# tbrown122387/ssme

Measured on AMD Instinct MI355X. Metric: particle-steps/sec (NxT) univ-SVOL bootstrap filter; log-lik delta vs CPU ref, higher is better.
Workload: dtype f64

## Files before the change

ssme_amd/csrc/pf_api.hip:

```cpp
#include "../../include/ssme_pf.h"
#include "pf_kernels.h"
#include "lw_kernels.h"
#include "pf_small.h"
#include "lw_small.h"
#include "user_expect.h"
#include "forecast.h"
#include "smooth.h"
#include "series_history.h"
#include "handle_core.h"
#include "shard_driver.h"

#include <cmath>
#include <cstdio>
#include <cstdlib>
#include <chrono>
#include <cstring>
#include <new>
#include <string>
#include <vector>

using namespace ssme;

struct StepKernels { const void* fn[2][2][3]; const void* wide[2]; int nt; };

struct ssme_pf_s : HandleCore {
    ssme_pf_config cfg;
    StepKernels kern;
    bool params_set;
    int debug_anc, keep_logw;
    int graph_mode;
    double *l2_T, *l2_R;
    double* l2_work;
    int32_t *l2_lo, *l2_hi;
    int32_t* l2_ticket;
    int l2_tables;
    double* small_ms;
    double* yz_step;
    int32_t* ticket;
    int num_cus;
    int small_series;
    double y_step_v[3];
    double z_step_v[3];
    int dx, dy;
    int kcov, kz;
    int nt;
    double *sh_x[2], *sh_c[2], *sh_loc, *sh_tsum, *sh_tmax, *sh_winx, *sh_winc;
    int sh_path;
    double* x[2];
    double* cdf[2];
    double* tsum[2];
    double* tmax[2];
    double *logw, *scratchR;
    double *exp_part, *exp_out;
    double* wscratch;
    double *uexp_part, *uexp_out;
    double last_z;
    double last_zv[kMaxCov];
    double* fc_zfut;
    size_t fc_zfut_cap;
    double *gam, *pgam, *gtot;
    uint32_t* anc;
    FilterScalars* scal;
    ModelConst* mc;
    int cur;
    hipGraphExec_t gexec;
    int g_T, g_has_z, g_debug, g_logw, g_nt;
    FunctionalIds g_rec_fs;
    int g_rec_user;
    FunctionalIds rec_fs;
    int rec_user;
    double *traj, *utraj;
    int traj_cap, traj_n;
    int rec_T, rec_n, rec_nh;
    SeriesHistoryState hist;
    double* hist_x;
    uint32_t* hist_anc;
// ... 162 lines not shown
                hipMemcpy(hs.data(), g_stamps, hs.size() * 8, hipMemcpyDeviceToHost);
                FILE* f = fopen(getenv("SSME_STAMPS_DUMP"), "w");
                for (size_t i = 0; i < hs.size(); i += 16) { for (int k = 0; k < 16; ++k) fprintf(f, "%llu ", hs[i + k]); fprintf(f, "\n"); }
                fclose(f);
            }
        }
    }
#endif
    return a;
}

static int default_tile(int n_particles, int n_filters) {
    if (n_particles <= kTile) return kTile;
    const long R = n_filters;
    if (R * ((n_particles + kTileSmall - 1) / kTileSmall) <= 256) return kTileSmall;
    if (R * ((n_particles + kTileMid - 1) / kTileMid) <= 512) return kTileMid;
    return kTile;
}

template <class F>
static void with_model(int model, F&& f) {
    switch (model) {
        case SSME_MODEL_SVOL: f(std::integral_constant<int, MODEL_SVOL>{}); break;
        case SSME_MODEL_SVOL_LEVERAGE: f(std::integral_constant<int, MODEL_SVOL_LEVERAGE>{}); break;
#if SSME_HAS_USER_MODEL
        case SSME_MODEL_USER0: f(std::integral_constant<int, MODEL_USER0>{}); break;
#endif
        default: f(std::integral_constant<int, MODEL_LIN_GAUSS>{}); break;
    }
}

template <int MODEL, int NT, int TILE, bool BIG, bool WL2>
static void fill_rs(const void* (&fn)[3]) {
    fn[0] = reinterpret_cast<const void*>(&k_filter_step<MODEL, NT, BIG, TILE, -1, WL2>);
    fn[1] = reinterpret_cast<const void*>(&k_filter_step<MODEL, NT, BIG, TILE, 0, WL2>);
    fn[2] = reinterpret_cast<const void*>(&k_filter_step<MODEL, NT, BIG, TILE, 1, WL2>);
}
template <int MODEL, int NT, int TILE>
static void fill_step_kernels(StepKernels& k) {
    k.nt = NT;
    fill_rs<MODEL, NT, TILE, false, false>(k.fn[0][0]);
    fill_rs<MODEL, NT, TILE, false, true>(k.fn[0][1]);
    fill_rs<MODEL, NT, TILE, true, false>(k.fn[1][0]);
}
template <int MODEL>
static StepKernels step_kernels(int tile) {
    StepKernels k{};
    if (tile == kTileSmall) fill_step_kernels<MODEL, 256, kTileSmall>(k);
    else if (tile == kTileMid) fill_step_kernels<MODEL, 512, kTileMid>(k);
    else {
        fill_step_kernels<MODEL, 512, kTile>(k);
        k.wide[0] = reinterpret_cast<const void*>(&k_filter_step<MODEL, 256, false, kTile, -1>);
        k.wide[1] = reinterpret_cast<const void*>(&k_filter_step<MODEL, 1024, false, kTile, -1>);
    }
    return k;
}
static hipError_t grant_step_lds(const ssme_pf_s* h) {
    hipError_t e = hipSuccess;
    for (int big = 0; big < 2; ++big)
        for (int wl2 = 0; wl2 < 2; ++wl2)
            for (const void* fn : h->kern.fn[big][wl2])
                if (fn && e == hipSuccess) e = grant_lds(fn, big ? h->lds_bytes_big : h->lds_bytes, h->cfg.device);
    for (const void* fn : h->kern.wide)
        if (fn && e == hipSuccess) e = grant_lds(fn, h->lds_bytes, h->cfg.device);
    return e;
}

struct StepLaunch { const void* fn; int nt; size_t lds; };
static StepLaunch select_step_kernel(const ssme_pf_s* h, const StepArgs& a) {
    int rs = -1;
    if (h->cfg.resamp_sched == 1 && a.t > 0 && !a.anc && !a.logw && !a.ticket)
        rs = h->cfg.resampler == SSME_RESAMP_MULTINOMIAL ? 0 : (h->cfg.resampler == SSME_RESAMP_SYSTEMATIC ? 1 : -1);
    if (h->split_l2) return {h->kern.fn[1][0][rs + 1], h->kern.nt, h->lds_bytes_big};
    if (h->tile == kTile && h->nt != 512) return {h->kern.wide[h->nt == 1024], h->nt, h->lds_bytes};
    return {h->kern.fn[0][a.B <= 128 ? 1 : 0][rs + 1], h->kern.nt, h->lds_bytes};
}
static void launch_step_on(ssme_pf_handle h, const StepArgs& a, dim3 grid) {
    const StepLaunch k = select_step_kernel(h, a);
    void* args[] = {const_cast<StepArgs*>(&a)};
    hipLaunchKernel(k.fn, grid, dim3(k.nt), args, k.lds, h->stream);
}
static void launch_step(ssme_pf_handle h, const StepArgs& a) { launch_step_on(h, a, dim3(h->B, h->R)); }
static void launch_gamma(ssme_pf_handle h, int t0, int nT) {
    if (h->cfg.resampler != SSME_RESAMP_MULTINOMIAL) return;
    launch_gamma_tables(h, h->gam, h->pgam, h->gtot, STREAM_GAMMA, STREAM_RESAMP_EXTRA, h->tile, h->cfg.first_filter_id, t0, nT);
}
static void launch_level2(hipStream_t st, const StepArgs& a, int n_filters, size_t lds, int ranges) {
    if (a.l2_inkernel) {
        hipLaunchKernelGGL(k_l2_scan_blocks, dim3((a.B + 1023) / 1024, n_filters), dim3(1024), 0, st, a);
    } else if (a.l2_work && a.B > 1024) {
        const dim3 grid((a.B + 1023) / 1024, n_filters);
        hipLaunchKernelGGL(k_l2_scan_blocks, grid, dim3(1024), 0, st, a);
        hipLaunchKernelGGL(k_l2_ranges, grid, dim3(1024), lds, st, a, ranges);
    } else
        hipLaunchKernelGGL(k_level2_plan, dim3(n_filters), dim3(1024), lds, st, a, ranges);
}
static void launch_plan(ssme_pf_handle h, int t, int gi, bool plan_ranges, bool finalize_prev, bool record_per_step,
                        double* ll_host = nullptr) {
    StepArgs a = step_args(h);
    a.t = t; a.gi = gi; a.finalize_prev = finalize_prev ? 1 : 0;
    a.ll_host = ll_host;
    a.per_step = record_per_step ? h->per_step : nullptr;
    launch_level2(h->stream, a, h->R, h->lds_bytes_plan, plan_ranges ? 1 : 0);
}
static void launch_kf(ssme_pf_handle h, int t, bool record_per_step, double* ll_host = nullptr) {
    if (h->split_l2) { launch_plan(h, t + 1, 0, false, true, record_per_step, ll_host); return; }
    StepArgs a = step_args(h);
    a.ll_host = ll_host;
    a.t = t;
    a.per_step = record_per_step ? h->per_step : nullptr;
    hipLaunchKernelGGL(kf_finalize, dim3(h->R), dim3(kThreads), 0, h->stream, a);
}

static double* hist_row(const ssme_pf_s* h, int t) { return h->hist_x + (size_t)t * h->dx * h->R * h->Npad; }

static void enqueue_step(ssme_pf_handle h, int t, int yi, int gi, bool has_z, bool finalize_prev, bool record_per_step,
                         bool from_step_staging = false, bool results_to_host = true) {
    StepArgs a = step_args(h);
    a.z = has_z ? h->zbuf : nullptr;
    if (from_step_staging) {
        a.by_value = 1; a.y_now = h->pin[PinLayout::yz]; a.z_now = has_z ? h->pin[PinLayout::yz + 1] : 0.0;
        for (int d = 1; d < h->dy; ++d) a.y_now_v[d - 1] = h->y_step_v[d - 1];
        for (int j = 1; j < h->kcov; ++j) a.z_now_v[j - 1] = has_z ? h->z_step_v[j - 1] : 0.0;
        if (!h->split_l2) { a.ticket = h->ticket; a.ll_host = results_to_host ? h->pin_dev + PinLayout::results : nullptr; }
    }
    a.per_step = record_per_step ? h->per_step : nullptr;
    a.t = t; a.yi = yi; a.gi = gi; a.finalize_prev = finalize_prev ? 1 : 0;
// ... 2265 lines not shown
```

ssme_amd/csrc/pf_kernels.h:

```cpp
#pragma once
#include "ssme_math.h"
#include "model_api.h"

namespace ssme {

typedef unsigned long long u64;

constexpr int kThreads = 256;
constexpr int kWave = 64;
constexpr int kRow = 512;
constexpr int kTile = 2048;
constexpr int kTileSmall = 512;
constexpr int kTileMid = 1024;
constexpr int kMaxTilesPerFilter = 2048;
constexpr int kSplitLevel2Above = 1024;
constexpr int kL2Scratch = 64;
constexpr int kL2Offsets = 32;
constexpr int kMaxTilesSplit = 16384;
#ifndef SSME_SEARCH_WINDOW
#define SSME_SEARCH_WINDOW 16
#endif
constexpr int kStageTiles = 3;
constexpr int kEShift = 35;
constexpr int kTileShift = 41;
// ... 60 lines not shown
    int32_t* l2_lo;
    int32_t* l2_hi;
    double* l2_work;
    int32_t l2_inkernel;
    int32_t* l2_ticket;
    const double* l2_tsrc;
    const double* l2_offs;
    int32_t l2_offs_stride;
    int32_t prio_mode;
    int32_t stream_stores;
    const uint32_t* keyp;
    uint32_t first_filter;
    double logN;
    int32_t ablate;
    unsigned long long* stamps;
};

template <int CTRL, int ROWMASK>
__device__ __forceinline__ double dpp_f64_neginf(double v) {
    const u64 b = d2bits(v);
    const int lo = __builtin_amdgcn_update_dpp(0, (int)(uint32_t)b, CTRL, ROWMASK, 0xF, false);
    const int hi = __builtin_amdgcn_update_dpp((int)0xfff00000, (int)(uint32_t)(b >> 32), CTRL, ROWMASK, 0xF, false);
    return bits2d(((u64)(uint32_t)hi << 32) | (u64)(uint32_t)lo);
}
template <int CTRL, int ROWMASK>
__device__ __forceinline__ double dpp_f64_zero(double v) {
    const u64 b = d2bits(v);
    int lo, hi;
    if (ROWMASK == 0xF) {
        lo = __builtin_amdgcn_mov_dpp((int)(uint32_t)b, CTRL, 0xF, 0xF, true);
        hi = __builtin_amdgcn_mov_dpp((int)(uint32_t)(b >> 32), CTRL, 0xF, 0xF, true);
    } else {
        lo = __builtin_amdgcn_update_dpp(0, (int)(uint32_t)b, CTRL, ROWMASK, 0xF, false);
        hi = __builtin_amdgcn_update_dpp(0, (int)(uint32_t)(b >> 32), CTRL, ROWMASK, 0xF, false);
    }
    return bits2d(((u64)(uint32_t)hi << 32) | (u64)(uint32_t)lo);
}
__device__ __forceinline__ double wave_incl_scan_f64(double v) {
    v = v + dpp_f64_zero<0x111, 0xF>(v);
    v = v + dpp_f64_zero<0x112, 0xF>(v);
    v = v + dpp_f64_zero<0x114, 0xF>(v);
    v = v + dpp_f64_zero<0x118, 0xF>(v);
    v = v + dpp_f64_zero<0x142, 0xA>(v);
    v = v + dpp_f64_zero<0x143, 0xC>(v);
    return v;
}
__device__ __forceinline__ double row16_incl_scan(double v) {
    v = v + dpp_f64_zero<0x111, 0xF>(v);
    v = v + dpp_f64_zero<0x112, 0xF>(v);
    v = v + dpp_f64_zero<0x114, 0xF>(v);
    v = v + dpp_f64_zero<0x118, 0xF>(v);
    return v;
}
__device__ __forceinline__ double wave_shr1_f64(double v) { return dpp_f64_zero<0x138, 0xF>(v); }
__device__ __forceinline__ double readlane_f64(double v, int lane) {
    const u64 b = d2bits(v);
    const uint32_t lo = (uint32_t)__builtin_amdgcn_readlane((int)(uint32_t)b, lane);
    const uint32_t hi = (uint32_t)__builtin_amdgcn_readlane((int)(uint32_t)(b >> 32), lane);
    return bits2d(((u64)hi << 32) | lo);
}
__device__ __forceinline__ double readfirstlane_f64(double v) {
    const u64 b = d2bits(v);
    const uint32_t lo = (uint32_t)__builtin_amdgcn_readfirstlane((int)(uint32_t)b);
    const uint32_t hi = (uint32_t)__builtin_amdgcn_readfirstlane((int)(uint32_t)(b >> 32));
    return bits2d(((u64)hi << 32) | lo);
}

__device__ __forceinline__ u64 readlane_u64(u64 v, int lane) {
    const uint32_t lo = (uint32_t)__builtin_amdgcn_readlane((int)(uint32_t)v, lane);
    const uint32_t hi = (uint32_t)__builtin_amdgcn_readlane((int)(uint32_t)(v >> 32), lane);
    return ((u64)hi << 32) | lo;
}

template <int CTRL>
__device__ __forceinline__ double dpp_f64_perm(double v) {
    const u64 b = d2bits(v);
    const int lo = __builtin_amdgcn_mov_dpp((int)(uint32_t)b, CTRL, 0xF, 0xF, true);
    const int hi = __builtin_amdgcn_mov_dpp((int)(uint32_t)(b >> 32), CTRL, 0xF, 0xF, true);
    return bits2d(((u64)(uint32_t)hi << 32) | (u64)(uint32_t)lo);
}
__device__ __forceinline__ double dmax_raw(double a, double b) {
    double d;
    asm("v_max_f64 %0, %1, %2" : "=v"(d) : "v"(a), "v"(b));
    return d;
}
__device__ __forceinline__ double wave_max_f64(double v) {
    v = dmax_raw(v, dpp_f64_perm<0xB1>(v));
    v = dmax_raw(v, dpp_f64_perm<0x4E>(v));
    v = dmax_raw(v, dpp_f64_perm<0x141>(v));
    v = dmax_raw(v, dpp_f64_perm<0x140>(v));
    v = dmax_raw(v, dpp_f64_neginf<0x142, 0xA>(v));
    v = dmax_raw(v, dpp_f64_neginf<0x143, 0xC>(v));
    return bits2d(readlane_u64(d2bits(v), 63));
}

template <int NT>
__device__ __forceinline__ double block_max_nanprop(double m, bool nan, double* lds) {
    constexpr int NW = NT / 64;
    m = wave_max_f64(m);
    const bool any = __ballot(nan) != 0;
    if ((threadIdx.x & 63) == 0) lds[threadIdx.x >> 6] = any ? dnan() : m;
    __syncthreads();
    double s[NW];
#pragma unroll
    for (int w = 0; w < NW; ++w) s[w] = lds[w];
    double r = s[0];
    bool un = false;
#pragma unroll
    for (int w = 1; w < NW; ++w) r = dmax_raw(r, s[w]);
#pragma unroll
    for (int w = 0; w < NW; w += 2) un = un || __builtin_isunordered(s[w], s[w + 1 < NW ? w + 1 : w]);
    return un ? dnan() : r;
}

template <int NT, int NK>
__device__ __forceinline__ void block_scan_f64(const double (&q)[NK][2], double (&incl)[NK][2], double& total, double* lds_seg) {
    constexpr int WPR = NT / 64, NSEG = NK * WPR;
    static_assert(NSEG <= 16, "segment totals are scanned inside one 16-lane row");
    const int lane = threadIdx.x & 63;
    const int wave = __builtin_amdgcn_readfirstlane(threadIdx.x >> 6);
    double s0[NK], s1[NK], exc[NK];
#pragma unroll
    for (int k = 0; k < NK; ++k) {
        s0[k] = q[k][0];
        s1[k] = s0[k] + q[k][1];
        const double inc = wave_incl_scan_f64(s1[k]);
        exc[k] = wave_shr1_f64(inc);
        if (lane == 63) lds_seg[k * WPR + wave] = inc;
    }
    __syncthreads();
    const double sv = row16_incl_scan((lane & 15) < NSEG ? lds_seg[lane & 15] : 0.0);
    total = readlane_f64(sv, 15);
#pragma unroll
    for (int k = 0; k < NK; ++k) {
        const int seg = k * WPR + wave;
        const double pre = seg ? readlane_f64(sv, seg - 1) : 0.0;
        const double base = pre + exc[k];
        incl[k][0] = base + s0[k];
        incl[k][1] = base + s1[k];
    }
}

template <int MODEL>
__device__ __forceinline__ double model_prop(const ModelConst& c, double x, double zn, double zcov, const ExpTabEntry* etab) {
#if SSME_HAS_USER_MODEL
    if constexpr (MODEL == MODEL_USER0) return user_calls<ssme_user_model0>::prop(c, x, zn, zcov, etab);
#endif
    if (MODEL == MODEL_SVOL_LEVERAGE) {
        const double e = dexp_scaled_t(-0.5 * x, 0, etab);
        const double mean = (c.a1 + c.a0 * (x - c.a1)) + (c.a4 * zcov) * e;
        return mean + zn * c.a3;
    }
    return c.a0 * x + zn * c.a1;
}

template <int MODEL>
__device__ __forceinline__ double model_logg(const ModelConst& c, double y, double x, const ExpTabEntry* etab) {
#if SSME_HAS_USER_MODEL
    if constexpr (MODEL == MODEL_USER0) return c.bad ? -dinf() : user_calls<ssme_user_model0>::logg(c, y, x, etab);
#endif
    if (MODEL == MODEL_LIN_GAUSS) {
        const double d = (y - x) * c.a4;
        const double v = (-c.a3 - SSME_HALF_LOG_2PI) - 0.5 * (d * d);
        return c.bad ? -dinf() : v;
    }
    const double logb = (MODEL == MODEL_SVOL) ? c.a3 : 0.0;
    const double ib2 = (MODEL == MODEL_SVOL) ? c.a4 : 1.0;
    const double hl = logb + 0.5 * x;
    const double e = dexp_scaled_t(-x, 0, etab);
    const double q = (y * y) * ib2;
    double v = (-hl - SSME_HALF_LOG_2PI) - 0.5 * (q * e);
    if (hl < -745.1332191019412) v = -dinf();
    if (MODEL == MODEL_SVOL && c.bad) v = -dinf();
    return v;
}

template <int MODEL>
__device__ __forceinline__ double scalar_step(const ModelConst& c, bool first_step, double x, double zn, double y, double zcov,
                                              const CovVals<model_kcov<MODEL>()>& zc, double* xn, const ExpTabEntry* etab) {
    if constexpr (model_kcov<MODEL>() > 0) {
#if SSME_HAS_USER_MODEL
        return cov_step<typename user_model_of<MODEL>::type>(c, first_step, &x, &zn, &y, zc.v, xn, etab);
#else
        return 0.0;
#endif
    } else {
        *xn = first_step ? zn * c.a2 : model_prop<MODEL>(c, x, zn, zcov, etab);
        return model_logg<MODEL>(c, y, *xn, etab);
    }
}

template <int MODEL>
// ... 183 lines not shown

__device__ __forceinline__ double systematic_u0(uint32_t t, uint32_t rep, uint32_t key0, uint32_t key1) {
    const u32x4 ox = philox4x32_10(0u, t, rep, STREAM_RESAMP_EXTRA, key0, key1);
    return u01_co(ox.v0, ox.v1);
}
__device__ __forceinline__ void draw_consts(const StepArgs& a, int resampler, int r, uint32_t rep, double& G, double& u0) {
    G = 1.0; u0 = 0.0;
    if (resampler == RESAMP_MULTINOMIAL) G = a.gtot[(size_t)a.gi * a.R + r];
    else if (resampler == RESAMP_SYSTEMATIC) u0 = systematic_u0((uint32_t)a.t, rep, a.keyp[0], a.keyp[1]);
}

__device__ __forceinline__ double lse_of(double m, double S, int rshift) {
    const double Sd = (S > 0.0) ? dldexp(S, -rshift) : dnan();
    return m + dlog(Sd);
}
__device__ __forceinline__ double account_step(FilterScalars* sc, double m, double S, int rshift, bool resampled, double logN) {
    const double lse = lse_of(m, S, rshift);
    const double ll = lse - sc->prev;
    sc->m = m;
    sc->S = S;
    sc->last_ll = ll;
    sc->loglik = sc->loglik + ll;
    sc->prev = resampled ? logN : lse;
    return ll;
}

template <int NT, int KMAX>
__device__ __forceinline__ void reg_max_nanflag(const double (&Mreg)[KMAX], int B, double& mx, bool& nan) {
    mx = -dinf();
    nan = false;
#pragma unroll
    for (int k = 0; k < KMAX; ++k) {
        if (k * NT + (int)threadIdx.x < B) { const double v = Mreg[k]; nan = nan || (v != v); mx = (v > mx) ? v : mx; }
    }
}

__device__ __forceinline__ void prio_at(int mode, int idx) {
    if (mode == 1) {
        if (idx == 0) __builtin_amdgcn_s_setprio(3); else if (idx == 3) __builtin_amdgcn_s_setprio(2);
        else if (idx == 6) __builtin_amdgcn_s_setprio(1); else if (idx == 8) __builtin_amdgcn_s_setprio(0);
    } else if (mode == 2) {
        if (idx == 0) __builtin_amdgcn_s_setprio(3); else if (idx == 3) __builtin_amdgcn_s_setprio(2);
        else if (idx == 5) __builtin_amdgcn_s_setprio(1); else if (idx == 6) __builtin_amdgcn_s_setprio(0);
    } else if (mode == 3) {
        if (idx == 0) __builtin_amdgcn_s_setprio(3); else if (idx == 4) __builtin_amdgcn_s_setprio(2);
        else if (idx == 7) __builtin_amdgcn_s_setprio(1); else if (idx == 9) __builtin_amdgcn_s_setprio(0);
    } else if (mode == 4) {
        if (idx == 0) __builtin_amdgcn_s_setprio(3); else if (idx == 2) __builtin_amdgcn_s_setprio(2);
        else if (idx == 4) __builtin_amdgcn_s_setprio(1); else if (idx == 6) __builtin_amdgcn_s_setprio(0);
    } else if (mode == 5) {
        if (idx == 0) __builtin_amdgcn_s_setprio(1); else if (idx == 6) __builtin_amdgcn_s_setprio(0);
    }
}
#define PRIO_AT(i) prio_at(a.prio_mode, i)

template <int STEP, int NQ>
struct lds_count_search {
    static __device__ __forceinline__ void run(uint32_t (&pa)[NQ], const double (&t)[NQ]) {
        static_assert(NQ == 1 || NQ == 2 || NQ == 4 || NQ == 8, "one to eight searches per thread");
        double v[NQ];
#pragma unroll
        for (int q = 0; q < NQ; ++q) asm volatile("ds_read_b64 %0, %1 offset:%2" : "=&v"(v[q]) : "v"(pa[q]), "n"((STEP - 1) * 8) : "memory");
        if constexpr (NQ == 8) asm volatile("s_waitcnt lgkmcnt(0)" : "+v"(v[0]), "+v"(v[1]), "+v"(v[2]), "+v"(v[3]), "+v"(v[4]), "+v"(v[5]), "+v"(v[6]), "+v"(v[7]));
        else if constexpr (NQ == 4) asm volatile("s_waitcnt lgkmcnt(0)" : "+v"(v[0]), "+v"(v[1]), "+v"(v[2]), "+v"(v[3]));
        else if constexpr (NQ == 2) asm volatile("s_waitcnt lgkmcnt(0)" : "+v"(v[0]), "+v"(v[1]));
        else asm volatile("s_waitcnt lgkmcnt(0)" : "+v"(v[0]));
#pragma unroll
        for (int q = 0; q < NQ; ++q) pa[q] = (v[q] < t[q]) ? pa[q] + (uint32_t)(STEP * 8) : pa[q];
        lds_count_search<STEP / 2, NQ>::run(pa, t);
    }
};
template <int NQ>
struct lds_count_search<0, NQ> {
    static __device__ __forceinline__ void run(uint32_t (&)[NQ], const double (&)[NQ]) {}
};

template <int TILE, int NK>
__device__ __forceinline__ void staged_search(const double (&tau)[NK][2], int span, double Pm, double T0, double T1, double R0, double R1,
                                              double R2, const double* lds_stage, int (&off)[NK][2]) {
    double tloc[NK][2];
    uint32_t pb[NK][2];
    typedef __attribute__((address_space(3))) const double lds_cdouble;
    const uint32_t stage_a = (uint32_t)(__UINTPTR_TYPE__)(lds_cdouble*)lds_stage;
    if (span == 1) {
#pragma unroll
        for (int k = 0; k < NK; ++k) {
#pragma unroll
            for (int c = 0; c < 2; ++c) { tloc[k][c] = __builtin_ceil((tau[k][c] - Pm) * R0); pb[k][c] = stage_a; }
        }
    } else if (span == 2) {
#pragma unroll
        for (int k = 0; k < NK; ++k) {
#pragma unroll
            for (int c = 0; c < 2; ++c) {
                const bool up = T0 < tau[k][c];
                tloc[k][c] = __builtin_ceil((tau[k][c] - (up ? T0 : Pm)) * (up ? R1 : R0));
                pb[k][c] = up ? stage_a + (uint32_t)(TILE * 8) : stage_a;
            }
        }
    } else {
#pragma unroll
        for (int k = 0; k < NK; ++k) {
#pragma unroll
            for (int c = 0; c < 2; ++c) {
                const double target = tau[k][c];
                int sel = (T0 < target ? 1 : 0) + (T1 < target ? 1 : 0);
                sel = sel < span - 1 ? sel : span - 1;
                const double Pb = sel == 0 ? Pm : (sel == 1 ? T0 : T1);
                const double Rb = sel == 0 ? R0 : (sel == 1 ? R1 : R2);
                tloc[k][c] = __builtin_ceil((target - Pb) * Rb);
                pb[k][c] = stage_a + (uint32_t)sel * (uint32_t)(TILE * 8);
            }
        }
    }
    if constexpr (SSME_SEARCH_WINDOW > 0 && NK >= 2) {
        constexpr int W = SSME_SEARCH_WINDOW > 0 ? SSME_SEARCH_WINDOW : 2;
        static_assert(W >= 2 && (W & (W - 1)) == 0 && W <= TILE, "the window is a power of two inside the tile");
        uint32_t pa0[NK], pa1[NK], top[NK];
        double t0[NK], t1[NK];
#pragma unroll
        for (int k = 0; k < NK; ++k) { pa0[k] = pb[k][0]; t0[k] = tloc[k][0]; t1[k] = tloc[k][1]; }
        lds_count_search<TILE / 2, NK>::run(pa0, t0);
#pragma unroll
        for (int k = 0; k < NK; ++k) {
            const uint32_t lo = pb[k][1], hi = pb[k][1] + (uint32_t)((TILE - W) * 8);
            const uint32_t st = pa0[k] > lo ? pa0[k] : lo;
            pa1[k] = st < hi ? st : hi;
            top[k] = pa1[k] + (uint32_t)((W - 1) * 8);
        }
        lds_count_search<W / 2, NK>::run(pa1, t1);
        bool open = false;
#pragma unroll
        for (int k = 0; k < NK; ++k) open = open || pa1[k] == top[k];
        if (__builtin_amdgcn_ballot_w64(open)) {
#pragma unroll
            for (int k = 0; k < NK; ++k) pa1[k] = pb[k][1];
            lds_count_search<TILE / 2, NK>::run(pa1, t1);
        }
#pragma unroll
        for (int k = 0; k < NK; ++k) { off[k][0] = (int)((pa0[k] - stage_a) >> 3); off[k][1] = (int)((pa1[k] - stage_a) >> 3); }
    } else {
        uint32_t pa[2 * NK];
        double tq[2 * NK];
#pragma unroll
        for (int k = 0; k < NK; ++k) { pa[2 * k] = pb[k][0]; pa[2 * k + 1] = pb[k][1]; tq[2 * k] = tloc[k][0]; tq[2 * k + 1] = tloc[k][1]; }
        lds_count_search<TILE / 2, 2 * NK>::run(pa, tq);
#pragma unroll
        for (int k = 0; k < NK; ++k) { off[k][0] = (int)((pa[2 * k] - stage_a) >> 3); off[k][1] = (int)((pa[2 * k + 1] - stage_a) >> 3); }
    }
}

__device__ __forceinline__ void clamp_to_window(int32_t* flag, int win_tile0, int win_tiles, int B, int& bb_min, int& span) {
    if (!flag) return;
    const int first = win_tile0 > 0 ? win_tile0 : 0, last = win_tile0 + win_tiles - 1 < B - 1 ? win_tile0 + win_tiles - 1 : B - 1;
    if (bb_min < first || bb_min + span - 1 > last) {
        if (threadIdx.x == 0) atomicOr(flag, 1);
        bb_min = bb_min < first ? first : (bb_min > last ? last : bb_min);
        span = 1;
    }
}

template <int NT>
__device__ __forceinline__ void publish_ratios(const double (&A)[2048 / NT], const double (&Ap)[2048 / NT], int B, int Bpow2, int bb_min,
                                               int span, double* R3, double* R_all) {
    constexpr int NE = 2048 / NT;
    const int tid = threadIdx.x;
    if (span <= kStageTiles) {
#pragma unroll
        for (int e = 0; e < NE; ++e) {
            if (e * NT < Bpow2) {
                const int j = e * NT + tid;
#pragma unroll
                for (int sl = 0; sl < kStageTiles; ++sl) {
                    const int bs = bb_min + sl < B ? bb_min + sl : B - 1;
                    if (j == bs) R3[sl] = A[e] / Ap[e];
                }
            }
        }
    } else {
#pragma unroll
        for (int e = 0; e < NE; ++e) {
            if (e * NT < Bpow2) {
                const int j = e * NT + tid;
                if (j < Bpow2) R_all[j] = (j < B) ? A[e] / Ap[e] : 0.0;
            }
        }
        __syncthreads();
    }
}

template <int NT, int NK, int TILE>
struct StagedTiles {
    double2 stg0[NK], stg1[NK], stg2[NK];
    __device__ __forceinline__ void load(const double* src, int span) {
#pragma unroll
        for (int k = 0; k < NK; ++k) { stg0[k] = make_double2(0.0, 0.0); stg1[k] = stg0[k]; stg2[k] = stg0[k]; }
        if (span > kStageTiles) return;
        const unsigned char* base = reinterpret_cast<const unsigned char*>(src);
        const uint32_t lane_off = (uint32_t)threadIdx.x * 16u;
#pragma unroll
        for (int k = 0; k < NK; ++k) stg0[k] = *reinterpret_cast<const double2*>(base + (lane_off + (uint32_t)(k * NT * 16)));
        if (span >= 2) {
// ... 32 lines not shown
        qe[k][1] = __builtin_rint(e1 * 34359738368.0);
        if (i_first + TILE > N) {
            asm volatile("");
            const int i0 = i_first + (k * NT + (int)threadIdx.x) * 2;
            if (!(i0 < N)) qe[k][0] = 0.0;
            if (!(i0 + 1 < N)) qe[k][1] = 0.0;
        }
    }
    block_scan_f64<NT, NK>(qe, le, se, lds_seg);
    const double ratio = gam / se;
#pragma unroll
    for (int k = 0; k < NK; ++k) {
#pragma unroll
        for (int c = 0; c < 2; ++c) {
            const double t1 = ratio * le[k][c];
            const double t2 = pgam + t1;
            tau[k][c] = __builtin_ceil(t2 * t_scale);
        }
    }
}

template <class TF>
__device__ __forceinline__ void staged_prefixes(TF Tof, int bb_min, int B, double& Pm, double& T0, double& T1) {
    T0 = Tof(bb_min);
    T1 = (bb_min + 1 < B) ? Tof(bb_min + 1) : dinf();
    Pm = bb_min ? Tof(bb_min - 1) : 0.0;
}
template <class RF>
__device__ __forceinline__ void staged_ratios(RF Rof, int bb_min, int B, double& R0, double& R1, double& R2) {
    const int b1 = bb_min + 1 < B ? bb_min + 1 : B - 1, b2 = bb_min + 2 < B ? bb_min + 2 : B - 1;
    R0 = Rof(bb_min); R1 = Rof(b1); R2 = Rof(b2);
}

template <class TF, class RF>
__device__ __forceinline__ int probe_ancestor(double target, TF Tof, RF Rof, const double* cdf_row, int B, int Bpow2, int tile,
                                              int win_tile0, int N) {
    int bb = count_less_pow2(Bpow2, target, Tof);
    bb = bb < B - 1 ? bb : B - 1;
    const double Pb = bb ? Tof(bb - 1) : 0.0;
    const double tloc = __builtin_ceil((target - Pb) * Rof(bb));
    const double* tl = cdf_row + (size_t)(bb - win_tile0) * tile;
    const int j = count_less_pow2(tile, tloc, [&](int q) { return tl[q]; });
    const int anc = bb * tile + j;
    return anc < N - 1 ? anc : N - 1;
}

typedef double f64x2_t __attribute__((ext_vector_type(2)));
__device__ __forceinline__ void store_pair(double* p, double v0, double v1, int stream) {
    if (stream) {
        f64x2_t v = {v0, v1};
        __builtin_nontemporal_store(v, reinterpret_cast<f64x2_t*>(p));
    } else *reinterpret_cast<double2*>(p) = make_double2(v0, v1);
}
template <int MODEL, int NT, bool BIG = false, int TILE = kTile, int RS = -1, bool WL2 = false>
__global__ __launch_bounds__(NT) void k_filter_step(const StepArgs a) {
    constexpr int NK = TILE / 2 / NT;
    constexpr bool HOT = RS >= 0;
    static_assert(NK >= 1 && NK * NT * 2 == TILE, "tile = 2 NT NK particles");
    extern __shared__ __attribute__((aligned(16))) unsigned char smem[];
    const int nT2 = (BIG || a.Bpow2 < 2) ? 2 : a.Bpow2;
    double* lds_stage = reinterpret_cast<double*>(smem);
    double* lds_T = lds_stage + kStageTiles * TILE;
    double* lds_R = lds_T + nT2;
    __shared__ double lds_seg_a[16];
    __shared__ double lds_seg_l2[64];
    __shared__ double lds_seg_c[16];
    __shared__ int lds_cnt[2];
    __shared__ double lds_R3[4];
    __shared__ double lds_d1[16];
    __shared__ double lds_d2[16];
    __shared__ __attribute__((aligned(16))) DrawTabs lds_dtab;
    __shared__ __attribute__((aligned(16))) ExpTabEntry lds_etab[SSME_EXP_TABLE_SIZE];

    const int tid = threadIdx.x;
    load_log_table<NT>(&lds_dtab);
    load_exp_table<NT>(lds_etab);
    const int gtile = xcd_tile_of_block((int)(blockIdx.x + gridDim.x * blockIdx.y), (int)(gridDim.x * gridDim.y));
    const int r = gtile / (int)gridDim.x, bloc = gtile - r * (int)gridDim.x;
    const int b = bloc + a.tile0;
    const int out0 = a.tile0 * TILE, win0 = a.win_tile0 * TILE;
    const uint32_t rep = a.first_filter + (uint32_t)r;
    const uint32_t key0 = a.keyp[0], key1 = a.keyp[1];
    const size_t rowoff = (size_t)r * a.Npad;
    const ModelConst mc = a.mc[r];
    constexpr int DX = model_dx<MODEL>(), DY = model_dy<MODEL>();
    constexpr bool VEC = DX > 1 || DY > 1;
    const double y = a.by_value ? a.y_now : a.y[(size_t)a.yi * DY];
    const double zcov = a.by_value ? a.z_now : (a.z ? a.z[a.yi] : 0.0);
    constexpr int KC = model_kcov<MODEL>();
    CovVals<KC> zc;
    if constexpr (KC > 0) {
#pragma unroll
        for (int j = 0; j < KC; ++j)
            zc.v[j] = a.by_value ? (j ? a.z_now_v[j > 0 ? j - 1 : 0] : a.z_now) : (a.z ? a.z[(size_t)a.yi * KC + j] : 0.0);
    }
    const int rsm = HOT ? RS : a.resampler;
    const bool first_step = !HOT && a.t == 0;
    const bool resampled = HOT ? true : ((a.t > 0) && (a.t % a.resamp_sched == 0));
    const bool need_l2 = HOT ? true : ((a.t > 0) && (resampled || (!BIG && bloc == 0 && a.finalize_prev)));
    const bool sorted = rsm != RESAMP_MULTINOMIAL_IID;
    uint32_t* const anc_p = HOT ? nullptr : a.anc;
    double* const logw_p = HOT ? nullptr : a.logw;
    const int i_first = b * TILE;
    const int nvalid = (a.N - i_first) < TILE ? (a.N - i_first) : TILE;
    const bool ragged = nvalid < TILE;

    STAMP(a, 0);
    PRIO_AT(0);
    constexpr int NE = 2048 / NT;
    double A2[NE], M2[NE], ApL2[NE];
// ... 154 lines not shown
    }
    STAMP(a, 4);
    PRIO_AT(4);

    double xin[NK][2], lw_old[NK][2];
    int srcv[NK][2];
#pragma unroll
    for (int k = 0; k < NK; ++k) { srcv[k][0] = 0; srcv[k][1] = 0; }
    if (first_step) {
#pragma unroll
        for (int k = 0; k < NK; ++k) { xin[k][0] = 0.0; xin[k][1] = 0.0; lw_old[k][0] = 0.0; lw_old[k][1] = 0.0; }
    } else if (!resampled) {
#pragma unroll
        for (int k = 0; k < NK; ++k) {
            const size_t idx = rowoff + (size_t)(i_first - out0) + (k * NT + tid) * 2;
            const double2 xv = *reinterpret_cast<const double2*>(a.x_in + idx);
            const double2 lv = *reinterpret_cast<const double2*>(logw_p + idx);
            xin[k][0] = xv.x; xin[k][1] = xv.y; lw_old[k][0] = lv.x; lw_old[k][1] = lv.y;
            if constexpr (DX > 1) { srcv[k][0] = i_first + (k * NT + tid) * 2; srcv[k][1] = srcv[k][0] + 1; }
        }
    } else {
        if (rsm != RESAMP_MULTINOMIAL) {
#pragma unroll
            for (int k = 0; k < NK; ++k) {
                const int i0 = i_first + (k * NT + tid) * 2;
                if (rsm == RESAMP_SYSTEMATIC) {
                    tau[k][0] = __builtin_ceil(((double)i0 + u0) * t_scale);
                    tau[k][1] = __builtin_ceil(((double)(i0 + 1) + u0) * t_scale);
                } else {
                    const u32x4 o = philox4x32_10((uint32_t)(i0 >> 1), (uint32_t)a.t, rep, STREAM_RESAMP, key0, key1);
                    const double v0 = u01_co(o.v0, o.v1), v1 = u01_co(o.v2, o.v3);
                    if (rsm == RESAMP_STRATIFIED) {
                        tau[k][0] = __builtin_ceil(((double)i0 + v0) * t_scale);
                        tau[k][1] = __builtin_ceil(((double)(i0 + 1) + v1) * t_scale);
                    } else {
                        tau[k][0] = __builtin_ceil(v0 * S);
                        tau[k][1] = __builtin_ceil(v1 * S);
                    }
                }
            }
        }

        auto Tof = [&](int j) -> double { return BIG ? l2Tg(j) : lds_T[j]; };
        auto Tinf = [&](int j) -> double { return BIG ? (j < a.B ? l2Tg(j) : dinf()) : lds_T[j]; };
        if (span <= kStageTiles) {
            stg.store(lds_stage, span);
            double Pm, T0, T1, R0, R1, R2;
            staged_prefixes(Tof, bb_min, a.B, Pm, T0, T1);
            __syncthreads();
            if (BIG) staged_ratios([&](int j) { return l2R[j]; }, bb_min, a.B, R0, R1, R2);
            else { R0 = lds_R3[0]; R1 = lds_R3[1]; R2 = lds_R3[2]; }
            STAMP(a, 5);
            PRIO_AT(5);
            int soff[NK][2];
            if (ABL(a, 2)) {
#pragma unroll
                for (int k = 0; k < NK; ++k) { soff[k][0] = (int)(d2bits(tau[k][0]) >> 20) & 2047; soff[k][1] = (int)(d2bits(tau[k][1]) >> 20) & 2047; }
            } else staged_search<TILE, NK>(tau, span, Pm, T0, T1, R0, R1, R2, lds_stage, soff);
            const unsigned char* xbase = reinterpret_cast<const unsigned char*>(xin_r - win0);
#pragma unroll
            for (int k = 0; k < NK; ++k) {
#pragma unroll
                for (int c = 0; c < 2; ++c) {
                    int anc = bb_min * TILE + soff[k][c];
                    anc = anc < a.N - 1 ? anc : a.N - 1;
                    const int i = i_first + (k * NT + tid) * 2 + c;
                    if (anc_p && i < a.N) anc_p[rowoff + i - out0] = (uint32_t)anc;
                    xin[k][c] = *reinterpret_cast<const double*>(xbase + ((uint32_t)anc << 3));
                    if constexpr (DX > 1) srcv[k][c] = anc;
                    lw_old[k][c] = 0.0;
                }
            }
        } else {
#pragma unroll
            for (int k = 0; k < NK; ++k) {
#pragma unroll
                for (int c = 0; c < 2; ++c) {
                    const int anc = probe_ancestor(tau[k][c], Tinf, [&](int j) { return BIG ? l2R[j] : lds_R[j]; }, cdf_r, a.B, a.Bpow2, TILE,
                                                   a.win_tile0, a.N);
                    const int i = i_first + (k * NT + tid) * 2 + c;
                    if (anc_p && i < a.N) anc_p[rowoff + i - out0] = (uint32_t)anc;
                    xin[k][c] = xin_r[anc - win0];
                    if constexpr (DX > 1) srcv[k][c] = anc;
                    lw_old[k][c] = 0.0;
                }
            }
        }
    }
    STAMP(a, 6);
    PRIO_AT(6);

    double zn[NK][2];
#pragma unroll
    for (int k = 0; k < NK; ++k) {
        if (ABL(a, 0)) { zn[k][0] = 0.25 + 1e-9 * (double)nw0[k]; zn[k][1] = -0.25; }
        else pair_normals(nw0[k], nw1[k], &lds_dtab, &zn[k][0], &zn[k][1]);
    }
    STAMP(a, 7);
    PRIO_AT(7);

    double lg[NK][2];
    double mx = -dinf();
    bool nan = false;
#pragma unroll
    for (int k = 0; k < NK; ++k) {
        const int i0 = i_first + (k * NT + tid) * 2;
        double xo[2];
        double xov[VEC ? kMaxDim : 1][2];
        if constexpr (VEC) {
#if SSME_HAS_USER_MODEL
            double yv[kMaxDim];
            yv[0] = y;
#pragma unroll
            for (int d = 1; d < DY; ++d) yv[d] = a.by_value ? a.y_now_v[d - 1] : a.y[(size_t)a.yi * DY + d];
            double znd[kMaxDim][2];
            znd[0][0] = zn[k][0]; znd[0][1] = zn[k][1];
#pragma unroll
            for (int d = 1; d < DX; ++d) {
                const u32x4 o = xdim_words((uint32_t)(b * (TILE / 2) + k * NT + tid), (uint32_t)a.t, rep, d, key0, key1);
                pair_normals(o.v0, o.v1, &lds_dtab, &znd[d][0], &znd[d][1]);
            }
#pragma unroll
            for (int c = 0; c < 2; ++c) {
                double xv[kMaxDim], zv[kMaxDim], xn[kMaxDim];
                xv[0] = xin[k][c];
#pragma unroll
                for (int d = 1; d < DX; ++d) xv[d] = first_step ? 0.0 : a.x_in[(size_t)d * a.xplane + rowoff + (size_t)srcv[k][c]];
#pragma unroll
                for (int d = 0; d < DX; ++d) zv[d] = znd[d][c];
                const double gv = vector_step<MODEL>(mc, first_step, xv, zv, yv, zcov, zc, xn, lds_etab);
                xo[c] = xn[0];
#pragma unroll
                for (int d = 1; d < DX; ++d) xov[d][c] = xn[d];
                lg[k][c] = lw_old[k][c] + gv;
            }
#endif
        } else {
#pragma unroll
        for (int c = 0; c < 2; ++c) {
            double xn, gv;
            if (KC == 0 && ABL(a, 3)) {
                xn = first_step ? zn[k][c] * mc.a2 : model_prop<MODEL>(mc, xin[k][c], zn[k][c], zcov, lds_etab);
                gv = -0.5 * xn * xn;
            } else gv = scalar_step<MODEL>(mc, first_step, xin[k][c], zn[k][c], y, zcov, zc, &xn, lds_etab);
            xo[c] = xn;
            lg[k][c] = lw_old[k][c] + gv;
        }
        }
        if (ragged) {
            asm volatile("");
#pragma unroll
            for (int c = 0; c < 2; ++c)
                if (!((i0 + c) < a.N)) {
                    xo[c] = 0.0; lg[k][c] = -dinf();
                    if constexpr (DX > 1) { for (int d = 1; d < DX; ++d) xov[d][c] = 0.0; }
                }
        }
#pragma unroll
        for (int c = 0; c < 2; ++c) { const double l = lg[k][c]; nan = nan || (l != l); mx = (l > mx) ? l : mx; }
        const size_t idx = rowoff + (size_t)(i0 - out0);
        store_pair(reinterpret_cast<double*>(reinterpret_cast<unsigned char*>(a.x_out + rowoff + (size_t)(i_first - out0)) + (uint32_t)(k * NT + tid) * 16u),
                   xo[0], xo[1], a.stream_stores);
        if (logw_p) *reinterpret_cast<double2*>(logw_p + idx) = make_double2(lg[k][0], lg[k][1]);
        if constexpr (DX > 1) {
#pragma unroll
            for (int d = 1; d < DX; ++d) *reinterpret_cast<double2*>(a.x_out + (size_t)d * a.xplane + idx) = make_double2(xov[d][0], xov[d][1]);
        }
    }
    STAMP(a, 8);
    PRIO_AT(8);
    const double mb = block_max_nanprop<NT>(mx, nan, lds_d2);
    STAMP(a, 9);
    PRIO_AT(9);

    double q[NK][2], inc[NK][2], total;
#pragma unroll
    for (int k = 0; k < NK; ++k) {
        if (ABL(a, 4)) { q[k][0] = (double)(d2bits(lg[k][0] - mb) >> 24); q[k][1] = (double)(d2bits(lg[k][1] - mb) >> 24); }
        else {
            q[k][0] = __builtin_rint(dexp_scaled_t(lg[k][0] - mb, kTileShift, lds_etab));
            q[k][1] = __builtin_rint(dexp_scaled_t(lg[k][1] - mb, kTileShift, lds_etab));
        }
    }
    if (ABL(a, 5)) {
#pragma unroll
        for (int k = 0; k < NK; ++k) { inc[k][0] = q[k][0]; inc[k][1] = q[k][0] + q[k][1]; }
        total = inc[0][1] + 1048576.0;
    } else block_scan_f64<NT, NK>(q, inc, total, lds_seg_c);
    STAMP(a, 12);
    PRIO_AT(12);
#pragma unroll
    for (int k = 0; k < NK; ++k) {
        store_pair(reinterpret_cast<double*>(reinterpret_cast<unsigned char*>(a.cdf_out + rowoff + (size_t)(i_first - out0)) + (uint32_t)(k * NT + tid) * 16u),
                   inc[k][0], inc[k][1], a.stream_stores);
    }
    STAMP(a, 10);
    PRIO_AT(10);
    bool fused_accounting = false;
    if constexpr (!HOT && !BIG) fused_accounting = a.ticket != nullptr;
    if (tid == 0) {
        double* ts = a.tsum_out + (size_t)r * a.Bs + (b - a.tile0);
        double* tm = a.tmax_out + (size_t)r * a.Bs + (b - a.tile0);
        if (fused_accounting) {
            __hip_atomic_store(ts, total, __ATOMIC_RELAXED, __HIP_MEMORY_SCOPE_AGENT);
            __hip_atomic_store(tm, mb, __ATOMIC_RELAXED, __HIP_MEMORY_SCOPE_AGENT);
        } else { *ts = total; *tm = mb; }
    }
    if constexpr (!HOT && !BIG) {
        if (fused_accounting) {
            __shared__ int lds_last;
            if (tid == 0) {
                int last = 1;
                if (gridDim.x > 1) {
                    asm volatile("s_waitcnt vmcnt(0)" ::: "memory");
                    last = __hip_atomic_fetch_add(a.ticket + r, 1, __ATOMIC_RELAXED, __HIP_MEMORY_SCOPE_AGENT) == (int)gridDim.x - 1;
                }
                lds_last = last;
            }
            __syncthreads();
            if (lds_last) {
                constexpr int NE2 = 2048 / NT;
                double A2[NE2], M2[NE2], Ap2[NE2], Tinc2[NE2], S2, m2;
#pragma unroll
                for (int e = 0; e < NE2; ++e) {
                    const int j = e * NT + tid;
                    A2[e] = 0.0; M2[e] = 0.0;
                    if (j < a.B) {
                        A2[e] = __hip_atomic_load(a.tsum_out + (size_t)r * a.Bs + j, __ATOMIC_RELAXED, __HIP_MEMORY_SCOPE_AGENT);
                        M2[e] = __hip_atomic_load(a.tmax_out + (size_t)r * a.Bs + j, __ATOMIC_RELAXED, __HIP_MEMORY_SCOPE_AGENT);
                    }
                }
                level2_scan<NT>(A2, M2, a.B, a.rshift, m2, Ap2, Tinc2, S2, lds_d1, lds_seg_l2, lds_etab);
                if (tid == 0) {
                    const double ll = account_step(a.scal + r, m2, S2, a.rshift, (a.t + 1) % a.resamp_sched == 0, a.logN);
                    if (a.per_step) a.per_step[(size_t)r * a.Tcap + a.t] = ll;
                    if (gridDim.x > 1) __hip_atomic_store(a.ticket + r, 0, __ATOMIC_RELAXED, __HIP_MEMORY_SCOPE_AGENT);
                    if (a.ll_host) a.ll_host[r] = ll;
                }
            }
        }
    }
#ifdef SSME_ABLATE
    __syncthreads();
    STAMP(a, 11);
    PRIO_AT(11);
#endif
}
// ... 453 lines not shown
```

Measured before the change: 86.42 billion.

## Add resident step kernel variant with wave-uniform staged search and simplified block scan

```diff
diff --git a/ssme_amd/csrc/pf_api.hip b/ssme_amd/csrc/pf_api.hip
--- a/ssme_amd/csrc/pf_api.hip
+++ b/ssme_amd/csrc/pf_api.hip
@@ -21,7 +21,7 @@
 
 using namespace ssme;
 
-struct StepKernels { const void* fn[2][2][3]; const void* wide[2]; int nt; };
+struct StepKernels { const void* fn[2][2][3]; const void* wide[2]; const void* resident[2]; int nt; };
 
 struct ssme_pf_s : HandleCore {
     ssme_pf_config cfg;
@@ -290,6 +290,8 @@
         fill_step_kernels<MODEL, 512, kTile>(k);
         k.wide[0] = reinterpret_cast<const void*>(&k_filter_step<MODEL, 256, false, kTile, -1>);
         k.wide[1] = reinterpret_cast<const void*>(&k_filter_step<MODEL, 1024, false, kTile, -1>);
+        k.resident[0] = reinterpret_cast<const void*>(&k_filter_step<MODEL, 512, false, kTile, 0, false, true>);
+        k.resident[1] = reinterpret_cast<const void*>(&k_filter_step<MODEL, 512, false, kTile, 1, false, true>);
     }
     return k;
 }
@@ -301,6 +303,8 @@
                 if (fn && e == hipSuccess) e = grant_lds(fn, big ? h->lds_bytes_big : h->lds_bytes, h->cfg.device);
     for (const void* fn : h->kern.wide)
         if (fn && e == hipSuccess) e = grant_lds(fn, h->lds_bytes, h->cfg.device);
+    for (const void* fn : h->kern.resident)
+        if (fn && e == hipSuccess) e = grant_lds(fn, h->lds_bytes, h->cfg.device);
     return e;
 }
 
@@ -311,6 +315,7 @@
         rs = h->cfg.resampler == SSME_RESAMP_MULTINOMIAL ? 0 : (h->cfg.resampler == SSME_RESAMP_SYSTEMATIC ? 1 : -1);
     if (h->split_l2) return {h->kern.fn[1][0][rs + 1], h->kern.nt, h->lds_bytes_big};
     if (h->tile == kTile && h->nt != 512) return {h->kern.wide[h->nt == 1024], h->nt, h->lds_bytes};
+    if (rs >= 0 && a.B > 128 && a.prio_mode == 1 && a.stream_stores == 1 && h->kern.resident[rs]) return {h->kern.resident[rs], h->kern.nt, h->lds_bytes};
     return {h->kern.fn[0][a.B <= 128 ? 1 : 0][rs + 1], h->kern.nt, h->lds_bytes};
 }
 static void launch_step_on(ssme_pf_handle h, const StepArgs& a, dim3 grid) {
diff --git a/ssme_amd/csrc/pf_kernels.h b/ssme_amd/csrc/pf_kernels.h
--- a/ssme_amd/csrc/pf_kernels.h
+++ b/ssme_amd/csrc/pf_kernels.h
@@ -136,7 +136,6 @@
     v = v + dpp_f64_zero<0x118, 0xF>(v);
     return v;
 }
-__device__ __forceinline__ double wave_shr1_f64(double v) { return dpp_f64_zero<0x138, 0xF>(v); }
 __device__ __forceinline__ double readlane_f64(double v, int lane) {
     const u64 b = d2bits(v);
     const uint32_t lo = (uint32_t)__builtin_amdgcn_readlane((int)(uint32_t)b, lane);
@@ -203,14 +202,11 @@
     static_assert(NSEG <= 16, "segment totals are scanned inside one 16-lane row");
     const int lane = threadIdx.x & 63;
     const int wave = __builtin_amdgcn_readfirstlane(threadIdx.x >> 6);
-    double s0[NK], s1[NK], exc[NK];
+    double inc[NK];
 #pragma unroll
     for (int k = 0; k < NK; ++k) {
-        s0[k] = q[k][0];
-        s1[k] = s0[k] + q[k][1];
-        const double inc = wave_incl_scan_f64(s1[k]);
-        exc[k] = wave_shr1_f64(inc);
-        if (lane == 63) lds_seg[k * WPR + wave] = inc;
+        inc[k] = wave_incl_scan_f64(q[k][0] + q[k][1]);
+        if (lane == 63) lds_seg[k * WPR + wave] = inc[k];
     }
     __syncthreads();
     const double sv = row16_incl_scan((lane & 15) < NSEG ? lds_seg[lane & 15] : 0.0);
@@ -219,9 +215,8 @@
     for (int k = 0; k < NK; ++k) {
         const int seg = k * WPR + wave;
         const double pre = seg ? readlane_f64(sv, seg - 1) : 0.0;
-        const double base = pre + exc[k];
-        incl[k][0] = base + s0[k];
-        incl[k][1] = base + s1[k];
+        incl[k][1] = pre + inc[k];
+        incl[k][0] = incl[k][1] - q[k][1];
     }
 }
 
@@ -511,7 +506,7 @@
         if (idx == 0) __builtin_amdgcn_s_setprio(1); else if (idx == 6) __builtin_amdgcn_s_setprio(0);
     }
 }
-#define PRIO_AT(i) prio_at(a.prio_mode, i)
+#define PRIO_AT(i) prio_at(RESIDENT ? 1 : a.prio_mode, i)
 
 template <int STEP, int NQ>
 struct lds_count_search {
@@ -534,41 +529,76 @@
     static __device__ __forceinline__ void run(uint32_t (&)[NQ], const double (&)[NQ]) {}
 };
 
+__device__ __forceinline__ uint32_t lds_addr(const double* p) {
+    typedef __attribute__((address_space(3))) const double lds_cdouble;
+    return (uint32_t)(__UINTPTR_TYPE__)(lds_cdouble*)p;
+}
 template <int TILE, int NK>
-__device__ __forceinline__ void staged_search(const double (&tau)[NK][2], int span, double Pm, double T0, double T1, double R0, double R1,
-                                              double R2, const double* lds_stage, int (&off)[NK][2]) {
+__device__ __forceinline__ void staged_search_pos(const double (&tau)[NK][2], int span, double Pm, double T0, double T1, double R0, double R1,
+                                                  double R2, const double* lds_stage, uint32_t (&pos)[NK][2]) {
     double tloc[NK][2];
     uint32_t pb[NK][2];
-    typedef __attribute__((address_space(3))) const double lds_cdouble;
-    const uint32_t stage_a = (uint32_t)(__UINTPTR_TYPE__)(lds_cdouble*)lds_stage;
-    if (span == 1) {
+    const uint32_t stage_a = lds_addr(lds_stage);
+    auto one_tile = [&](double P, double R, uint32_t base) {
 #pragma unroll
         for (int k = 0; k < NK; ++k) {
 #pragma unroll
-            for (int c = 0; c < 2; ++c) { tloc[k][c] = __builtin_ceil((tau[k][c] - Pm) * R0); pb[k][c] = stage_a; }
-        }
-    } else if (span == 2) {
+            for (int c = 0; c < 2; ++c) { tloc[k][c] = __builtin_ceil((tau[k][c] - P) * R); pb[k][c] = base; }
+        }
+    };
+    if (span == 1) one_tile(Pm, R0, stage_a);
+    else if (span == 2) {
+        bool any_up = false, all_up = true;
 #pragma unroll
         for (int k = 0; k < NK; ++k) {
 #pragma unroll
+            for (int c = 0; c < 2; ++c) { const bool up = T0 < tau[k][c]; any_up = any_up || up; all_up = all_up && up; }
+        }
+        if (!__builtin_amdgcn_ballot_w64(any_up)) {
+            asm volatile("");
+            one_tile(Pm, R0, stage_a);
+        } else if (!__builtin_amdgcn_ballot_w64(!all_up)) {
+            asm volatile("");
+            one_tile(T0, R1, stage_a + (uint32_t)(TILE * 8));
+        } else {
+#pragma unroll
+            for (int k = 0; k < NK; ++k) {
+#pragma unroll
+                for (int c = 0; c < 2; ++c) {
+                    const bool up = T0 < tau[k][c];
+                    tloc[k][c] = __builtin_ceil((tau[k][c] - (up ? T0 : Pm)) * (up ? R1 : R0));
+                    pb[k][c] = up ? stage_a + (uint32_t)(TILE * 8) : stage_a;
+                }
+            }
+        }
+    } else {
+        int sel[NK][2];
+        bool differs = false;
+#pragma unroll
+        for (int k = 0; k < NK; ++k) {
+#pragma unroll
             for (int c = 0; c < 2; ++c) {
-                const bool up = T0 < tau[k][c];
-                tloc[k][c] = __builtin_ceil((tau[k][c] - (up ? T0 : Pm)) * (up ? R1 : R0));
-                pb[k][c] = up ? stage_a + (uint32_t)(TILE * 8) : stage_a;
-            }
-        }
-    } else {
-#pragma unroll
-        for (int k = 0; k < NK; ++k) {
-#pragma unroll
-            for (int c = 0; c < 2; ++c) {
-                const double target = tau[k][c];
-                int sel = (T0 < target ? 1 : 0) + (T1 < target ? 1 : 0);
-                sel = sel < span - 1 ? sel : span - 1;
-                const double Pb = sel == 0 ? Pm : (sel == 1 ? T0 : T1);
-                const double Rb = sel == 0 ? R0 : (sel == 1 ? R1 : R2);
-                tloc[k][c] = __builtin_ceil((target - Pb) * Rb);
-                pb[k][c] = stage_a + (uint32_t)sel * (uint32_t)(TILE * 8);
+                const int s = (T0 < tau[k][c] ? 1 : 0) + (T1 < tau[k][c] ? 1 : 0);
+                sel[k][c] = s < span - 1 ? s : span - 1;
+            }
+        }
+        const int sel_u = __builtin_amdgcn_readfirstlane(sel[0][0]);
+#pragma unroll
+        for (int k = 0; k < NK; ++k) differs = differs || sel[k][0] != sel_u || sel[k][1] != sel_u;
+        if (!__builtin_amdgcn_ballot_w64(differs)) {
+            asm volatile("");
+            one_tile(sel_u == 0 ? Pm : (sel_u == 1 ? T0 : T1), sel_u == 0 ? R0 : (sel_u == 1 ? R1 : R2), stage_a + (uint32_t)sel_u * (uint32_t)(TILE * 8));
+        } else {
+#pragma unroll
+            for (int k = 0; k < NK; ++k) {
+#pragma unroll
+                for (int c = 0; c < 2; ++c) {
+                    const int s = sel[k][c];
+                    const double Pb = s == 0 ? Pm : (s == 1 ? T0 : T1);
+                    const double Rb = s == 0 ? R0 : (s == 1 ? R1 : R2);
+                    tloc[k][c] = __builtin_ceil((tau[k][c] - Pb) * Rb);
+                    pb[k][c] = stage_a + (uint32_t)s * (uint32_t)(TILE * 8);
+                }
             }
         }
     }
@@ -597,7 +627,7 @@
             lds_count_search<TILE / 2, NK>::run(pa1, t1);
         }
 #pragma unroll
-        for (int k = 0; k < NK; ++k) { off[k][0] = (int)((pa0[k] - stage_a) >> 3); off[k][1] = (int)((pa1[k] - stage_a) >> 3); }
+        for (int k = 0; k < NK; ++k) { pos[k][0] = pa0[k]; pos[k][1] = pa1[k]; }
     } else {
         uint32_t pa[2 * NK];
         double tq[2 * NK];
@@ -605,8 +635,17 @@
         for (int k = 0; k < NK; ++k) { pa[2 * k] = pb[k][0]; pa[2 * k + 1] = pb[k][1]; tq[2 * k] = tloc[k][0]; tq[2 * k + 1] = tloc[k][1]; }
         lds_count_search<TILE / 2, 2 * NK>::run(pa, tq);
 #pragma unroll
-        for (int k = 0; k < NK; ++k) { off[k][0] = (int)((pa[2 * k] - stage_a) >> 3); off[k][1] = (int)((pa[2 * k + 1] - stage_a) >> 3); }
-    }
+        for (int k = 0; k < NK; ++k) { pos[k][0] = pa[2 * k]; pos[k][1] = pa[2 * k + 1]; }
+    }
+}
+template <int TILE, int NK>
+__device__ __forceinline__ void staged_search(const double (&tau)[NK][2], int span, double Pm, double T0, double T1, double R0, double R1,
+                                              double R2, const double* lds_stage, int (&off)[NK][2]) {
+    uint32_t pos[NK][2];
+    staged_search_pos<TILE, NK>(tau, span, Pm, T0, T1, R0, R1, R2, lds_stage, pos);
+    const uint32_t stage_a = lds_addr(lds_stage);
+#pragma unroll
+    for (int k = 0; k < NK; ++k) { off[k][0] = (int)((pos[k][0] - stage_a) >> 3); off[k][1] = (int)((pos[k][1] - stage_a) >> 3); }
 }
 
 __device__ __forceinline__ void clamp_to_window(int32_t* flag, int win_tile0, int win_tiles, int B, int& bb_min, int& span) {
@@ -745,10 +784,11 @@
         __builtin_nontemporal_store(v, reinterpret_cast<f64x2_t*>(p));
     } else *reinterpret_cast<double2*>(p) = make_double2(v0, v1);
 }
-template <int MODEL, int NT, bool BIG = false, int TILE = kTile, int RS = -1, bool WL2 = false>
+template <int MODEL, int NT, bool BIG = false, int TILE = kTile, int RS = -1, bool WL2 = false, bool RESIDENT = false>
 __global__ __launch_bounds__(NT) void k_filter_step(const StepArgs a) {
     constexpr int NK = TILE / 2 / NT;
     constexpr bool HOT = RS >= 0;
+    static_assert(!RESIDENT || HOT, "the compiled-in schedule exists for the RS >= 0 kernels only");
     static_assert(NK >= 1 && NK * NT * 2 == TILE, "tile = 2 NT NK particles");
     extern __shared__ __attribute__((aligned(16))) unsigned char smem[];
     const int nT2 = (BIG || a.Bpow2 < 2) ? 2 : a.Bpow2;
@@ -1009,22 +1049,32 @@
             else { R0 = lds_R3[0]; R1 = lds_R3[1]; R2 = lds_R3[2]; }
             STAMP(a, 5);
             PRIO_AT(5);
-            int soff[NK][2];
+            uint32_t spos[NK][2];
             if (ABL(a, 2)) {
 #pragma unroll
-                for (int k = 0; k < NK; ++k) { soff[k][0] = (int)(d2bits(tau[k][0]) >> 20) & 2047; soff[k][1] = (int)(d2bits(tau[k][1]) >> 20) & 2047; }
-            } else staged_search<TILE, NK>(tau, span, Pm, T0, T1, R0, R1, R2, lds_stage, soff);
+                for (int k = 0; k < NK; ++k)
+                    for (int c = 0; c < 2; ++c) spos[k][c] = lds_addr(lds_stage) + (((uint32_t)(d2bits(tau[k][c]) >> 20) & 2047u) << 3);
+            } else staged_search_pos<TILE, NK>(tau, span, Pm, T0, T1, R0, R1, R2, lds_stage, spos);
             const unsigned char* xbase = reinterpret_cast<const unsigned char*>(xin_r - win0);
+            const uint32_t pos2byte = (uint32_t)bb_min * (uint32_t)(TILE * 8) - lds_addr(lds_stage);
+            const bool last_src_ragged = bb_min + span >= a.B && a.B * TILE > a.N;
+            uint32_t goff[NK][2];
+#pragma unroll
+            for (int k = 0; k < NK; ++k) { goff[k][0] = spos[k][0] + pos2byte; goff[k][1] = spos[k][1] + pos2byte; }
+            if (last_src_ragged) {
+                asm volatile("");
+                const uint32_t top = (uint32_t)(a.N - 1) << 3;
+#pragma unroll
+                for (int k = 0; k < NK; ++k) { goff[k][0] = goff[k][0] < top ? goff[k][0] : top; goff[k][1] = goff[k][1] < top ? goff[k][1] : top; }
+            }
 #pragma unroll
             for (int k = 0; k < NK; ++k) {
 #pragma unroll
                 for (int c = 0; c < 2; ++c) {
-                    int anc = bb_min * TILE + soff[k][c];
-                    anc = anc < a.N - 1 ? anc : a.N - 1;
                     const int i = i_first + (k * NT + tid) * 2 + c;
-                    if (anc_p && i < a.N) anc_p[rowoff + i - out0] = (uint32_t)anc;
-                    xin[k][c] = *reinterpret_cast<const double*>(xbase + ((uint32_t)anc << 3));
-                    if constexpr (DX > 1) srcv[k][c] = anc;
+                    if (anc_p && i < a.N) anc_p[rowoff + i - out0] = goff[k][c] >> 3;
+                    xin[k][c] = *reinterpret_cast<const double*>(xbase + goff[k][c]);
+                    if constexpr (DX > 1) srcv[k][c] = (int)(goff[k][c] >> 3);
                     lw_old[k][c] = 0.0;
                 }
             }
@@ -1117,7 +1167,7 @@
         for (int c = 0; c < 2; ++c) { const double l = lg[k][c]; nan = nan || (l != l); mx = (l > mx) ? l : mx; }
         const size_t idx = rowoff + (size_t)(i0 - out0);
         store_pair(reinterpret_cast<double*>(reinterpret_cast<unsigned char*>(a.x_out + rowoff + (size_t)(i_first - out0)) + (uint32_t)(k * NT + tid) * 16u),
-                   xo[0], xo[1], a.stream_stores);
+                   xo[0], xo[1], RESIDENT ? 1 : a.stream_stores);
         if (logw_p) *reinterpret_cast<double2*>(logw_p + idx) = make_double2(lg[k][0], lg[k][1]);
         if constexpr (DX > 1) {
 #pragma unroll
@@ -1149,7 +1199,7 @@
 #pragma unroll
     for (int k = 0; k < NK; ++k) {
         store_pair(reinterpret_cast<double*>(reinterpret_cast<unsigned char*>(a.cdf_out + rowoff + (size_t)(i_first - out0)) + (uint32_t)(k * NT + tid) * 16u),
-                   inc[k][0], inc[k][1], a.stream_stores);
+                   inc[k][0], inc[k][1], RESIDENT ? 1 : a.stream_stores);
     }
     STAMP(a, 10);
     PRIO_AT(10);
```

Result: faster. 89.24 billion (median of 6 runs) (+3.3%).
